# sholtodouglas/RoboticsPlayroomPybullet

Measured on AMD Instinct MI355X. Metric: env-steps/sec at N=4096 parallel UR5PlayAbsRPY1Obj-v0 envs per MI355X, higher is better.
Workload: dtype f32

## Files before the change

### roboticsplayroompybullet_amd/csrc/rp_kernels.cuh

```cuda
#pragma once
#include <hip/hip_runtime.h>
#include <stdint.h>

#include "rp_device_model.h"
#include "rp_math.cuh"

#define NB_MAX (1 + RP_MAX_ARM + RP_MAX_FREE + RP_MAX_J1)
#define NVP 28
#define MAXC 21
#define MAXACT 64
#define MAXT 4
#define MAXROWC (3 * MAXC + MAXT)
static_assert(MAXACT <= 64 && NB_MAX <= 32, "a candidate record packs its pair index in 6 bits and its bodies in 5 bits each");
#define PM_MAX 11
#define PMC_HDR 4
#define PMC_PT 11
#define PMC_MAN (8 + 4 * PMC_PT)
#define PMC_MANIFOLDS (PMC_HDR + PM_MAX * PMC_MAN)
#define PMC_AX PMC_MANIFOLDS
#define PMC_AXN 16
#define PMC_FLOATS (PMC_MANIFOLDS + 8 * PMC_AXN)
#define RP_MAX_GROUPS 16
#define SORT_KEYS 64
#define SORT_REPS 8
#define SORT_BINS (SORT_KEYS * SORT_REPS)
#define SORT_RANK_BITS 22
#define SORT_RANK_MASK ((1 << SORT_RANK_BITS) - 1)
#define RP_MAX_ENVS (1 << SORT_RANK_BITS)
#define MAXSMALL 44

#ifndef RP_PREP_WAVES
#define RP_PREP_WAVES 4
#endif
// ... 116 lines not shown
  };
  HULL_POOL_FIELDS
#ifdef RP_LDS_PAD
  float pad[RP_LDS_PAD];
#endif
};
static_assert(offsetof(EnvLds, aabb) % 16 == 0 && offsetof(PrepLds, aabb) % 16 == 0 && offsetof(EnvLds, cand) % 16 == 0 && offsetof(EnvLds, man) % 16 == 0 && offsetof(EnvLds, srow) % 16 == 0 && offsetof(EnvLds, rowS) % 16 == 0 &&
              offsetof(EnvLds, rowT) % 16 == 0 && offsetof(EnvLds, J) % 16 == 0 && offsetof(EnvLds, B) % 16 == 0, "16-byte LDS accesses");
static_assert(sizeof(PrepLds) <= 20480 - 512, "k_prep2: eight blocks (sixteen waves: what its 128 VGPRs allow) per CU");
static_assert(offsetof(PrepLds, roff) % 16 == 0 && offsetof(PrepLds, slot) % 16 == 0 && offsetof(PrepLds, Minv) % 16 == 0 && offsetof(PrepLds, aout) % 16 == 0 &&
              offsetof(PrepLds, Md) % 8 == 0 && offsetof(PrepLds, cand) % 16 == 0 && offsetof(PrepLds, man) % 16 == 0, "16-byte copies out of LDS");
static_assert(offsetof(PrepLds, rowS) % 16 == 0 && offsetof(PrepLds, rowT) % 16 == 0 && offsetof(PrepLds, J) % 8 == 0 && offsetof(PrepLds, B) % 8 == 0 && ROWW % 2 == 0,
              "prep2_core copies rowS / rowT a row (16 bytes) and J / B a pair (8 bytes) at a time");

struct __align__(16) ObsLds {
  float st[RP_REC_FLOATS];
  float xR[NB_MAX * 9], xp[NB_MAX * 3];
  float O[4];
  float S[RP_MAX_ARM * 6];
  alignas(16) float cand[2 * 12 * RP_MAX_ARM + 2 * RP_MAX_ARM + 4];
  alignas(16) float out[O_FLOATS];
};
#ifdef RP_CLOCKS
__device__ unsigned long long g_clk[32 * 4096];
#define CLK_MARK(i) if (lane == 0) { g_clk[8 * wb + (i)] = __builtin_readcyclecounter(); }
#if RP_CLOCKS == 2
#define PCLK(i) if (lane == 0) { g_clk[32 * (blockIdx.x & 4095) + (i)] = (i) >= 6 && (i) < 8 ? wall_clock64() : __builtin_readcyclecounter(); }
#define PCLK_ZERO(i) if (lane == 0) { g_clk[32 * (blockIdx.x & 4095) + (i)] = 0ull; }
#define PCLK_ADD(i, v) if (lane == 0) { g_clk[32 * (blockIdx.x & 4095) + (i)] += (unsigned long long)(v); }
#define HCLK_ADD(i, v) if (l16 == 0) { atomicAdd(&g_clk[32 * (blockIdx.x & 4095) + (i)], (unsigned long long)(v)); }
#ifdef RP_HPROF
#define PCLK_G(i, v)
#define PCLK_H(i, v) PCLK_ADD(i, v)
#else
#define PCLK_G(i, v) PCLK_ADD(i, v)
#define PCLK_H(i, v)
#endif
#define CLK_MARK2(i)
#else
#define PCLK(i)
#define PCLK_ZERO(i)
#define PCLK_ADD(i, v)
#define HCLK_ADD(i, v)
#define PCLK_G(i, v)
#define PCLK_H(i, v)
#define CLK_MARK2(i) CLK_MARK(i)
#endif
#else
#define CLK_MARK(i)
#define CLK_MARK2(i)
#define PCLK(i)
#define PCLK_ZERO(i)
#define PCLK_ADD(i, v)
#define HCLK_ADD(i, v)
#define PCLK_G(i, v)
#define PCLK_H(i, v)
#endif

#define WSYNC() do { __builtin_amdgcn_fence(__ATOMIC_RELEASE, "workgroup"); __builtin_amdgcn_wave_barrier(); __builtin_amdgcn_fence(__ATOMIC_ACQUIRE, "workgroup"); } while (0)

__device__ __forceinline__ int dof_free(const DevModel* m, int k) { return m->n_arm + 6 * k; }
__device__ __forceinline__ int dof_j1(const DevModel* m, int k) { return m->n_arm + 6 * m->n_free + k; }
#ifndef RP_WIDE
#define LANE_J1 16
#define LANE_FREE 19
__device__ __forceinline__ int lane_pos(const DevModel* m, int d) {
  if (d < m->n_arm) return d;
  const int e = d - m->n_arm, f6 = 6 * m->n_free;
  if (e >= f6) return LANE_J1 + (e - f6);
  const int f = e / 6, c = e - 6 * f;
  if ((m->free_row0 >> f) & 1) return c < 3 ? m->n_arm + c : -1;
  return LANE_FREE + e;
}
__device__ __forceinline__ int lane_dof(const DevModel* m, int l) {
  if (l < 16) {
    if (l < m->n_arm) return l;
// ... 70 lines not shown
  return x ^ (x >> 31);
}
__device__ __forceinline__ float rng_uniform(uint64_t seed, uint32_t env, uint32_t counter) {
  uint64_t h = splitmix64(seed ^ splitmix64(((uint64_t)env << 32) | counter));
  return (float)(h >> 40) * (1.0f / 16777216.0f);
}

struct Xf { M3 R; V3 p; };

__device__ __forceinline__ Xf joint_compose(const DevModel* m, const Xf& P, int j, float q) {
  Xf r;
  M3 Rj = mul(P.R, ldm3(m->arm_jrot[j]));
  r.p = P.p + mulv(P.R, ld3(m->arm_jpos[j]));
  V3 ax = ld3(m->arm_axis[j]);
  if (m->arm_jtype[j] == 0) {
    r.R = mul(Rj, axis_angle(ax, q));
  } else {
    r.R = Rj;
    r.p = r.p + mulv(Rj, ax) * q;
  }
  return r;
}

template <class LDS>
__device__ __forceinline__ void fk_bodies(const DevModel* m, LDS& L, int lane) {
  float* T = L.cand;
  static_assert(2 * 12 * RP_MAX_ARM + 2 * RP_MAX_ARM <= CANDMAX * 8 && 2 * 12 * RP_MAX_ARM + 2 * RP_MAX_ARM <= (int)(sizeof(L.cand) / sizeof(float)), "fk scratch fits the candidate list");
  int* P = (int*)(T + 2 * 12 * RP_MAX_ARM);
  const int n = m->n_arm;
  Xf x; x.R = ident3(); x.p = mk3(0, 0, 0);
  int par = -1;
  if (lane < n) {
    M3 R0 = ldm3(m->arm_jrot[lane]);
    V3 p0 = ld3(m->arm_jpos[lane]), ax = ld3(m->arm_axis[lane]);
    float q = L.st[ST_Q + lane];
    x.R = R0; x.p = p0;
    if (m->arm_jtype[lane] == 0) x.R = mul(R0, axis_angle(ax, q));
    else x.p = p0 + mulv(R0, ax) * q;
    par = m->arm_parent[lane];
    if (par < 0) { M3 Rb = ldm3(m->base_rot); V3 pb = ld3(m->base_pos); x.p = pb + mulv(Rb, x.p); x.R = mul(Rb, x.R); }
  }
  if (lane < m->nbody && !(lane >= 1 && lane <= n)) {
    int b = lane;
    Xf y; y.R = ident3(); y.p = mk3(0, 0, 0);
    if (b > n && b <= n + m->n_free) {
      int k = b - 1 - n;
      const float* f = &L.st[ST_FREE + 13 * k];
      Q4 q = {f[3], f[4], f[5], f[6]};
      y.R = quat_to_m3(q); y.p = ld3(f);
    } else if (b > n + m->n_free) {
      int k = b - 1 - n - m->n_free;
      M3 R0 = ldm3(m->j1_rot[k]);
      V3 ax = ld3(m->j1_axis[k]);
      y.p = ld3(m->j1_pos[k]);
      float q = L.st[ST_JQ + k];
      if (m->j1_type[k] == 0) y.R = mul(R0, axis_angle(ax, q));
      else { y.R = R0; y.p = y.p + mulv(R0, ax) * q; }
    }
    stm3(&L.xR[9 * b], y.R); st3(&L.xp[3 * b], y.p);
  }
  for (int it = 0; __ballot(par >= 0) != 0ull; it++) {
    float* Tb = T + (it & 1) * 12 * RP_MAX_ARM;
    int* Pb = P + (it & 1) * RP_MAX_ARM;
    if (lane < n) { stm3(&Tb[12 * lane], x.R); st3(&Tb[12 * lane + 9], x.p); Pb[lane] = par; }
    WSYNC();
    if (par >= 0) {
      M3 Ra = ldm3(&Tb[12 * par]); V3 pa = ld3(&Tb[12 * par + 9]);
      x.p = pa + mulv(Ra, x.p); x.R = mul(Ra, x.R);
      par = Pb[par];
    }
  }
  if (lane < n) { stm3(&L.xR[9 * (lane + 1)], x.R); st3(&L.xp[3 * (lane + 1)], x.p); }
}

template <class LDS>
__device__ __forceinline__ void joint_subspaces(const DevModel* m, LDS& L, int lane) {
  if (lane == 0) st3(L.O, ld3(&L.xp[3 * m->site_body[RP_SITE_EE]]));
  WSYNC();
  if (lane < m->n_arm) {
    V3 O = ld3(L.O);
    M3 R = ldm3(&L.xR[9 * (1 + lane)]);
    V3 a = mulv(R, ld3(m->arm_axis[lane]));
    V6 S;
    if (m->arm_jtype[lane] == 0) { S.a = a; S.l = cross(ld3(&L.xp[3 * (1 + lane)]) - O, a); }
    else { S.a = mk3(0, 0, 0); S.l = a; }
    st6(&L.S[6 * lane], S);
  }
}

template <class LDS>
__device__ __forceinline__ void stage_dynamics(const DevModel* m, LDS& L, int t, int env) {
  const int no = m->n_obj, nd = no + m->n_free;
  if (t < nd) {
    const float v = m->dyn[(size_t)env * nd + t];
    if (t < no) L.dmu[t] = v; else L.dmass[t - no] = v;
  }
}
template <class LDS>
__device__ __forceinline__ float pair_friction(const DevModel* m, const LDS& L, int a, int b) {
  return fminf(L.dmu[m->col_obj[a]] * L.dmu[m->col_obj[b]], 10.f);
}
__device__ __forceinline__ V3 ld_wrench(const DevModel* m, int env, int body, int half) {
  return ld3(m->wrench + ((size_t)env * (m->nbody - 1) + body) * 6 + 3 * half);
}
__device__ __forceinline__ bool wrench_on(V3 w) { return w.x != 0.f || w.y != 0.f || w.z != 0.f; }
__device__ __forceinline__ V3 ld_gravity(const DevModel* m, int env) { return ld3(m->act + (size_t)env * (3 + 2 * m->n_arm)); }
__device__ __forceinline__ float ld_motor_gain(const DevModel* m, int env, int dof) { return m->act[(size_t)env * (3 + 2 * m->n_arm) + 3 + dof]; }
__device__ __forceinline__ float ld_motor_strength(const DevModel* m, int env, int dof) { return m->act[(size_t)env * (3 + 2 * m->n_arm) + 3 + m->n_arm + dof]; }
template <class LDS>
__device__ __forceinline__ Xf collider_xf(const DevModel* m, const LDS& L, int c) {
  int b = m->col_body[c];
  M3 Rb = ldm3(&L.xR[9 * b]);
  Xf x;
  x.R = mul(Rb, ldm3(m->col_rot[c]));
  x.p = ld3(&L.xp[3 * b]) + mulv(Rb, ld3(m->col_pos[c]));
  return x;
}

template <class LDS>
__device__ __forceinline__ void collider_aabbs(const DevModel* m, LDS& L, int lane) {
  if (lane < m->n_col) {
    Xf x = collider_xf(m, L, lane);
    V3 he = ld3(m->col_he[lane]);
    float e[3];
    for (int i = 0; i < 3; i++)
      e[i] = m->col_type[lane] == 0 ? fabsf(x.R.m[3 * i]) * he.x + fabsf(x.R.m[3 * i + 1]) * he.y + fabsf(x.R.m[3 * i + 2]) * he.z : he.x;
    *(float4*)&L.aabb[8 * lane] = make_float4(x.p.x - e[0], x.p.y - e[1], x.p.z - e[2], m->col_margin[lane]);
    *(float4*)&L.aabb[8 * lane + 4] = make_float4(x.p.x + e[0], x.p.y + e[1], x.p.z + e[2], 0.f);
  }
}

struct CPt { V3 p, n; float dist; };

__device__ __forceinline__ int sphere_box(V3 cs, float r, V3 cb, const M3& Rb, V3 hb, float margin, int sphere_is_b, CPt* out) {
  const V3 l = tmulv(Rb, cs - cb);
  V3 cl = l;
  bool inside = true;
  if (cl.x > hb.x) { cl.x = hb.x; inside = false; }
  if (cl.x < -hb.x) { cl.x = -hb.x; inside = false; }
  if (cl.y > hb.y) { cl.y = hb.y; inside = false; }
  if (cl.y < -hb.y) { cl.y = -hb.y; inside = false; }
  if (cl.z > hb.z) { cl.z = hb.z; inside = false; }
  if (cl.z < -hb.z) { cl.z = -hb.z; inside = false; }
  V3 nl; float dist;
  if (!inside) {
    const V3 df = cl - l;
    const float len = norm(df);
    dist = len - r;
    if (dist > margin) return 0;
    nl = df * (1.f / len);
  } else {
    const float px = hb.x - fabsf(l.x), py = hb.y - fabsf(l.y), pz = hb.z - fabsf(l.z);
// ... 616 lines not shown
          pt.p = pB + nrm * (0.5f * dcon); pt.n = flip ? -nrm : nrm; pt.dist = dcon;
        }
        if (l16 == 0) {
          L.hout[gi] = out;
          if (out == 1) {
            float* q = &L.hpt[gi][0];
            st3(q, pt.p); st3(q + 3, pt.n); q[6] = pt.dist;
          }
        }
  }
}

template <class LDS>
__device__ __forceinline__ int narrowphase_coop(const DevModel* m, LDS& L, int lane, int nact, float* __restrict__ gax) {
  const int g = lane >> 3, s = lane & 7;
  float* scr = &L.npscr[NPG_SCRATCH * g];
  float* sv = scr;
  float (*poly)[8][3] = (float (*)[8][3])(scr + 16);
  float (*kept)[4] = (float (*)[4])(scr + 64);
  const unsigned below = (1u << s) - 1u;
  {
    const int ai = lane;
    const bool act = ai < nact;
    const int pi = act ? L.act[ai] : 0;
    const int a = m->pair[pi][0], b = m->pair[pi][1];
    const int ta = m->col_type[a], tb = m->col_type[b];
    const float margin0 = fminf(m->col_margin[a], m->col_margin[b]);
    int hf = -1;
      const int body_b0 = m->col_body[b], body_a0 = m->col_body[a];
      const bool hswap = act && m->hull_cnt[b] > 0 && ta == 0 && tb == 0 && body_a0 > m->n_arm;
      const int hc = hswap ? b : a, bc = hswap ? a : b;
      const int hn = act ? m->hull_cnt[hc] : 0;
      bool hq = hn > 0 && (hswap || (tb == 0 && body_b0 == 0));
      if (hq) {
        const Xf xa = collider_xf(m, L, hc), xb = collider_xf(m, L, bc);
        const V3 ha = ld3(m->col_he[hc]), hb0 = ld3(m->col_he[bc]);
        const V3 hb = mk3(fmaxf(hb0.x, RP_HULL_MARGIN), fmaxf(hb0.y, RP_HULL_MARGIN), fmaxf(hb0.z, RP_HULL_MARGIN));
        const V3 tt = xa.p - xb.p;
        const V3 A0 = col(xa.R, 0), A1 = col(xa.R, 1), A2 = col(xa.R, 2), B0 = col(xb.R, 0), B1 = col(xb.R, 1), B2 = col(xb.R, 2);
        const float r0 = ha.x * fabsf(dot(B0, A0)) + ha.y * fabsf(dot(B0, A1)) + ha.z * fabsf(dot(B0, A2));
        const float r1 = ha.x * fabsf(dot(B1, A0)) + ha.y * fabsf(dot(B1, A1)) + ha.z * fabsf(dot(B1, A2));
        const float r2 = ha.x * fabsf(dot(B2, A0)) + ha.y * fabsf(dot(B2, A1)) + ha.z * fabsf(dot(B2, A2));
        const float og = fmaxf(fmaxf(fabsf(dot(B0, tt)) - r0 - hb.x, fabsf(dot(B1, tt)) - r1 - hb.y), fabsf(dot(B2, tt)) - r2 - hb.z);
        const float q0 = hb.x * fabsf(dot(A0, B0)) + hb.y * fabsf(dot(A0, B1)) + hb.z * fabsf(dot(A0, B2));
        const float q1 = hb.x * fabsf(dot(A1, B0)) + hb.y * fabsf(dot(A1, B1)) + hb.z * fabsf(dot(A1, B2));
        const float q2 = hb.x * fabsf(dot(A2, B0)) + hb.y * fabsf(dot(A2, B1)) + hb.z * fabsf(dot(A2, B2));
        const float og2 = fmaxf(fmaxf(fabsf(dot(A0, tt)) - q0 - ha.x, fabsf(dot(A1, tt)) - q1 - ha.y), fabsf(dot(A2, tt)) - q2 - ha.z);
        if (fmaxf(og, og2) > margin0 + RP_HULL_MARGIN + 1e-5f) { hq = false; hf = 0; }
      }
      if (act) L.hout[ai] = hf;
      if (hq) { L.hinfo[ai][0] = hc | (bc << 8) | (hswap ? 65536 : 0); L.hinfo[ai][1] = __float_as_int(margin0); L.hinfo[ai][2] = pi; }
      const unsigned long long any = __ballot(hq);
      if (any != 0ull) {
        PCLK_H(30, -(long long)__builtin_readcyclecounter())
        const int slot = (gax && m->gjk) ? (pi & (PMC_AXN - 1)) : (ai & (PMC_AXN - 1));
        unsigned leaders = 0u;
        unsigned long long mycls = 0ull;
#pragma unroll 1
        for (int c = 0; c < PMC_AXN; c++) {
          const unsigned long long mk = __ballot(hq && slot == c);
          if (mk != 0ull) leaders |= 1u << c;
          if (lane == c) mycls = mk;
        }
        if (lane < PMC_AXN) L.hcls[lane] = mycls;
        WSYNC();
        {
          const int row = lane >> 4;
#pragma unroll 1
          for (unsigned rest = leaders; rest != 0u;) {
            unsigned t = rest;
            if (row >= 1) t &= t - 1u;
            if (row >= 2) t &= t - 1u;
            if (row >= 3) t &= t - 1u;
            unsigned long long cm = t != 0u ? L.hcls[__ffs(t) - 1] : 0ull;
            rest &= rest - 1u; rest &= rest - 1u; rest &= rest - 1u; rest &= rest - 1u;
#pragma unroll 1
            while (__any(cm != 0ull)) {
              const int gi = cm != 0ull ? __ffsll((long long)cm) - 1 : -1;
              cm &= cm - 1ull;
              hull_item16(m, L, lane, gi, gax);
            }
          }
        }
        PCLK_H(30, __builtin_readcyclecounter())
      }
    WSYNC();
    PCLK(19)
  }
  int cbase = 0;
  for (int base = 0; base < nact; base += 64 / NPG) {
    const int ai = base + g;
    const bool act = ai < nact;
    const int pi = act ? L.act[ai] : 0;
    const int a = m->pair[pi][0], b = m->pair[pi][1];
    const int ta = m->col_type[a], tb = m->col_type[b];
    const float margin0 = fminf(m->col_margin[a], m->col_margin[b]);
    const bool bbox = act && ta == 0 && tb == 0;
    if (act && s == 0) {
      const int n = m->n_arm, ba = m->col_body[a], bdy = m->col_body[b];
      const int kf = ba - 1 - n;
      const bool single = kf >= 0 && kf < m->n_free && m->free_rot_locked[kf] && bdy == 0;
      auto half0 = [&](int q) { int f = q - 1 - n; return q >= 1 && (q <= n || (f < m->n_free && ((m->free_row0 >> f) & 1))); };
      const bool r0 = half0(ba) || half0(bdy), r1 = (ba >= 1 && !half0(ba)) || (bdy >= 1 && !half0(bdy));
      const bool arm = (ba >= 1 && ba <= n) || (bdy >= 1 && bdy <= n), movable = ba > n || bdy > n;
      L.key[ai] = m->col_obj[a] * 256 + m->col_obj[b] + (single ? 65536 : 0) + ((r0 ? (r1 ? 2 : 1) : 0) << 20) + ((arm && movable) ? (1 << 22) : 0);
      L.pmu[ai] = pair_friction(m, L, a, b);
    }
    const int hf = act ? L.hout[ai] : -1;
    int np = 0;
    CPt mine; mine.p = mk3(0, 0, 0); mine.n = mk3(0, 0, 0); mine.dist = 0.f;
    if (hf == 1 && s == 0) { const float* hp = &L.hpt[ai][0]; mine.p = ld3(hp); mine.n = ld3(hp + 3); mine.dist = hp[6]; np = 1; }
    asm volatile("" ::: "memory");
    const Xf xa = collider_xf(m, L, a), xb = collider_xf(m, L, b);
    const V3 ha = ld3(m->col_he[a]), hb = ld3(m->col_he[b]);
    const bool bb = bbox && hf < 0;
    const int body_a = m->col_body[a], body_b = m->col_body[b];
    const bool arm_pair = (body_a >= 1 && body_a <= m->n_arm) || (body_b >= 1 && body_b <= m->n_arm);
    const float margin = (bb && (arm_pair || m->persist) && m->boxbox_margin >= 0.f) ? m->boxbox_margin : margin0;
    if (act && !bb && s == 0) {
      if (ta == 0 && tb == 1) np = sphere_box(xb.p, hb.x, xa.p, xa.R, ha, margin, 1, &mine);
      else if (ta == 1 && tb == 0) np = sphere_box(xa.p, ha.x, xb.p, xb.R, hb, margin, 0, &mine);
    }
    const V3 ca = xa.p, cb = xb.p;
    const V3 A0 = col(xa.R, 0), A1 = col(xa.R, 1), A2 = col(xa.R, 2), B0 = col(xb.R, 0), B1 = col(xb.R, 1), B2 = col(xb.R, 2);
    const V3 t = ca - cb;
    auto axis = [&](int ax, bool& valid) {
      valid = true;
      if (ax < 3) return pick3(ax, A0, A1, A2);
      if (ax < 6) return pick3(ax - 3, B0, B1, B2);
      int e = ax - 6, i = e / 3, j = e - 3 * i;
      V3 c = cross(pick3(i, A0, A1, A2), pick3(j, B0, B1, B2));
      float l = norm(c);
      valid = !(l < 1e-6f);
      return c * (1.f / l);
    };
#pragma unroll
    for (int round = 0; round < 2; round++) {
      int ax = 8 * round + s;
      if (bb && ax < 15) {
        bool valid;
        V3 Lx = axis(ax, valid);
        float ra = 0.f, rb = 0.f;
        ra += ha.x * fabsf(dot(Lx, A0)); rb += hb.x * fabsf(dot(Lx, B0));
        ra += ha.y * fabsf(dot(Lx, A1)); rb += hb.y * fabsf(dot(Lx, B1));
        ra += ha.z * fabsf(dot(Lx, A2)); rb += hb.z * fabsf(dot(Lx, B2));
        float sval = fabsf(dot(t, Lx)) - ra - rb;
        sv[ax] = valid ? sval : -1e30f;
      }
    }
    WSYNC();
    bool reject = !bb;
    float best_s = -1e30f, edge_s = -1e30f; int best_f = 0, ee = 0;
    if (bb) {
#pragma unroll
      for (int f = 0; f < 6; f++) {
        float sf = sv[f];
        reject |= sf > margin;
        if (sf > best_s + (f == 0 ? 0.f : K_TIE_EPS)) { best_s = sf; best_f = f; }
      }
#pragma unroll
      for (int e = 0; e < 9; e++) {
        float se = sv[6 + e];
        reject |= se > margin;
        if (se > edge_s + K_TIE_EPS) { edge_s = se; ee = e; }
      }
    }
    const bool live = bb && !reject;
    const bool edge_case = live && edge_s > best_s + 0.05f * fabsf(best_s) + 1e-6f;
    const bool face_case = live && !edge_case;
    const int best_kind = best_f < 3 ? 0 : 1, best_i = best_f < 3 ? best_f : best_f - 3;
    if (edge_case && s == 0) {
// ... 161 lines not shown
  return best;
}

__device__ __forceinline__ int solver_place(const int kept, const int pk, const unsigned long long lower, int& cls, int& before) {
  int key = 0, total = 0;
  cls = 0; before = 0;
  if (kept > 0) { cls = (pk >> 20) & 3; key = 2 * (cls == 2 ? 1 : 0) + ((pk >> 22) & 1); }
  unsigned long long mk[4];
#pragma unroll
  for (int k = 0; k < 4; k++) mk[k] = __ballot(kept > 0 && key == k);
#pragma unroll
  for (int bit = 0; bit < 3; bit++) {
    const unsigned long long mb = __ballot((kept >> bit) & 1);
    total += __popcll(mb) << bit;
#pragma unroll
    for (int k = 0; k < 4; k++) {
      const int all = __popcll(mb & mk[k]) << bit, low = __popcll(mb & mk[k] & lower) << bit;
      before += k < key ? all : (k == key ? low : 0);
    }
  }
  return total;
}

template <class LDS>
__device__ __forceinline__ int collide(const DevModel* m, LDS& L, int lane, int env, const int* npm_early = nullptr) {
  int nact = 0;
  const int npair = m->n_pair;
  const unsigned short* pp = (const unsigned short*)m->pair;
  unsigned short pv[RP_MAX_PAIR / 64];
#pragma unroll
  for (int k = 0; k < RP_MAX_PAIR / 64; k++) { int pi = 64 * k + lane; pv[k] = pp[pi < npair ? pi : 0]; }
  unsigned ovbits = 0u;
#pragma unroll
  for (int k = 0; k < RP_MAX_PAIR / 64; k++) {
    int pi = 64 * k + lane;
    if (64 * k < npair && pi < npair) {
      int a = pv[k] & 255, b = pv[k] >> 8;
      const float4 alo = *(const float4*)&L.aabb[8 * a], ahi = *(const float4*)&L.aabb[8 * a + 4];
      const float4 blo = *(const float4*)&L.aabb[8 * b], bhi = *(const float4*)&L.aabb[8 * b + 4];
      const float margin = fminf(alo.w, blo.w);
      bool sep = (alo.x > bhi.x + margin) | (blo.x > ahi.x + margin) | (alo.y > bhi.y + margin) | (blo.y > ahi.y + margin) | (alo.z > bhi.z + margin) | (blo.z > ahi.z + margin);
      ovbits |= sep ? 0u : (1u << k);
    }
  }
#pragma unroll
  for (int k = 0; k < RP_MAX_PAIR / 64; k++) {
    if (64 * k >= npair) break;
    bool ov = (ovbits >> k) & 1u;
    unsigned long long mask = __ballot(ov);
    int before = __popcll(mask & ((1ull << lane) - 1ull));
    if (ov && nact + before < MAXACT) L.act[nact + before] = 64 * k + lane;
    nact += __popcll(mask);
    if (nact >= MAXACT) { nact = MAXACT; break; }
  }
  WSYNC();
  PCLK(8)
#if defined(RP_CLOCKS) && RP_CLOCKS == 2
  if (lane == 0) g_clk[32 * (blockIdx.x & 4095) + 12] = nact;
#endif
  const int ncand_all = uni(narrowphase_coop<LDS>(m, L, lane, nact, m->persist ? m->pmcache + (size_t)env * PMC_FLOATS + PMC_AX : nullptr));
  WSYNC();
  asm volatile("" : "+v"(lane));
  PCLK(9)
  const unsigned long long lower = (1ull << lane) - 1ull;
  int kept = 0, pk = 0, total = 0;
  float* man = L.man;
  if (m->persist) {
    float* C = L.npscr + 8 * MANPTS;
    static_assert(8 * MANPTS + PMC_MANIFOLDS <= NPSCR_FLOATS, "the staged contact cache lies behind L.man in the narrowphase scratch");
    float* g = m->pmcache + (size_t)env * PMC_FLOATS;
    const int npm_pre = min(max(uni(npm_early ? *npm_early : __float_as_int(g[0])), 0), PM_MAX);
    const int used_in = PMC_HDR + PMC_MAN * npm_pre;
    for (int i = lane * 4; i < used_in; i += 256) *(float4*)&C[i] = *(const float4*)&g[i];
    if (lane == 0) C[0] = __int_as_float(npm_pre);
    WSYNC();
    PCLK(21)
    int npm = uni(__float_as_int(C[0]));
    const int mykey = lane < npm ? __float_as_int(C[PMC_HDR + PMC_MAN * lane]) : -1;
    const int akey = L.key[lane < nact ? lane : 0];
    const int pkey = L.key[lane >= 1 && lane < nact ? lane - 1 : 0];
    bool steady;
// ... 14 lines not shown
    }
    if (!steady) {
      {
        WSYNC();
        int nk = 0;
        for (int j = 0; j < npm; j++)
          if ((keep >> j) & 1ull) {
            if (nk != j && lane < PMC_MAN) C[PMC_HDR + PMC_MAN * nk + lane] = C[PMC_HDR + PMC_MAN * j + lane];
            nk++;
          }
        npm = nk;
        WSYNC();
      }
      {
        const int objk = lane < nact ? (L.key[lane] & 0xFFFF) : -1;
        const bool first = lane < nact && (lane == 0 || (L.key[lane - 1] & 0xFFFF) != objk);
        const int mkey = __float_as_int(C[PMC_HDR + PMC_MAN * (lane < npm ? lane : 0)]);
        bool present = false;
        for (int j = 0; j < npm; j++) present |= __builtin_amdgcn_readlane(mkey, j) == objk;
        const bool isnew = first && !present;
        const unsigned long long mnew = __ballot(isnew);
        const int slot = npm + __popcll(mnew & lower);
        if (isnew && slot < PM_MAX) {
          const int pi = L.act[lane];
          float* M = &C[PMC_HDR + PMC_MAN * slot];
          M[0] = __int_as_float(objk); M[1] = __int_as_float(0);
          M[2] = fminf(m->col_margin[m->pair[pi][0]], m->col_margin[m->pair[pi][1]]);
          M[3] = __int_as_float(L.key[lane] >> 16);
          for (int t = 4; t < PMC_MAN; t++) M[t] = 0.f;
        }
        npm = min(PM_MAX, npm + (int)__popcll(mnew));
        WSYNC();
      }
    }
    PCLK(22)
    unsigned long long unmatched, mine = 0ull;
    {
      const int ncand = ncand_all;
      const bool isc = lane < ncand;
      const float* c = &L.cand[8 * (isc ? lane : 0)];
      const V3 p = ld3(c), nr = mk3(c[3], c[4], c[5]);
      const float dist = c[6];
      const int abw = __float_as_int(c[7]);
      const int objk = L.key[(abw >> 16) & 63] & 0xFFFF;
      const int ba = (abw >> 22) & 31, bb = (abw >> 27) & 31;
      const M3 RA = ldm3(&L.xR[9 * ba]), RB = ldm3(&L.xR[9 * bb]);
      const V3 xA = ld3(&L.xp[3 * ba]), xB = ld3(&L.xp[3 * bb]);
      const int mkey = steady ? mykey : __float_as_int(C[PMC_HDR + PMC_MAN * (lane < npm ? lane : 0)]);
      int mi = -1;
      for (int jm = 0; jm < npm; jm++) if (__builtin_amdgcn_readlane(mkey, jm) == objk) mi = jm;
// ... 178 lines not shown
        } else if (cnt < 4) dst = cnt++;
        else dst = manifold_replace_index(man, c);
        if (dst >= 0) { const float4 c0 = *(const float4*)c, c1 = *(const float4*)(c + 4); *(float4*)&man[8 * dst] = c0; *(float4*)&man[8 * dst + 4] = c1; }
      }
    }
  }
  WSYNC();
  int cls, before;
  total = solver_place(kept, pk, lower, cls, before);
  for (int i = 0; i < kept; i++) {
    const float4 c0 = *(const float4*)&man[8 * i], c1 = *(const float4*)&man[8 * i + 4];
    const int ab = __float_as_int(c1.w);
    const int o = before + i;
    L.conp[3 * o] = c0.x; L.conp[3 * o + 1] = c0.y; L.conp[3 * o + 2] = c0.z;
    L.conn[3 * o] = c0.w; L.conn[3 * o + 1] = c1.x; L.conn[3 * o + 2] = c1.y;
    L.cond[o] = c1.z;
    L.cona[o] = ab & 255; L.conb[o] = (ab >> 8) & 255; L.conk[o] = cls;
    L.conmu[o] = L.pmu[(ab >> 16) & 63];
  }
  }
  WSYNC();
  PCLK(10)
  return total;
}

template <class LDS>
__device__ __forceinline__ void arm_dynamics(const DevModel* m, LDS& L, int lane, int env) {
  int n = m->n_arm;
  V3 O = ld3(L.O);
  V3 wf = mk3(0, 0, 0), wt = mk3(0, 0, 0);
  if (lane < n) { wf = ld_wrench(m, env, lane, 0); wt = ld_wrench(m, env, lane, 1); }
  const V3 grav = ld_gravity(m, env);
  if (lane < n) {
    M3 R = ldm3(&L.xR[9 * (1 + lane)]);
    V3 c = ld3(&L.xp[3 * (1 + lane)]) + mulv(R, ld3(m->arm_com[lane])) - O;
    float mass = m->arm_mass[lane];
    M3 Ic = ldm3(m->arm_inertia[lane]);
    M3 Rt; for (int i = 0; i < 3; i++) for (int j = 0; j < 3; j++) Rt.m[3 * i + j] = R.m[3 * j + i];
    M3 Iw = mul(mul(R, Ic), Rt);
    float cc = dot(c, c);
    float* I = &L.inert[10 * lane];
    I[0] = mass; st3(I + 1, c * mass);
    I[4] = Iw.m[0] + mass * (cc - c.x * c.x); I[5] = Iw.m[4] + mass * (cc - c.y * c.y); I[6] = Iw.m[8] + mass * (cc - c.z * c.z);
    I[7] = Iw.m[1] - mass * c.x * c.y; I[8] = Iw.m[2] - mass * c.x * c.z; I[9] = Iw.m[5] - mass * c.y * c.z;
  }
  WSYNC();
// ... 1490 lines not shown
#define W3_B (W3_J + ROWREG)
#define W3_SROW (W3_B + ROWREG)
#define W3_FLOATS (W3_SROW + 4 + 8 * MAXSMALL)
#define STAGE_FLOATS (128 + 2 * ROWREG)
#define AOUT_FLOATS (160 + 8 + 20)
static_assert(W3_A % 4 == 0 && W3_ROWS % 4 == 0 && W3_ROWT % 4 == 0 && W3_ROFF % 4 == 0 && AOUT_FLOATS % 4 == 0 && W3_FLOATS % 4 == 0, "16-byte copies");
static_assert(W3_J % 2 == 0 && W3_B % 2 == 0, "8-byte copies of the compact rows");

#define HV_MAXC 14
#ifndef S4_SLOTS0
#define S4_SLOTS0 8
#endif
#ifndef S4_SLOTS1
#define S4_SLOTS1 8
#endif
__device__ __forceinline__ int hv_class(int nc, int nA, int nB, int nC) {
  const bool heavy = nC != 0 || nA > S4_SLOTS0 || nB > S4_SLOTS1;
  return !heavy ? 0 : (nc <= HV_MAXC ? 1 : 2);
}
#define PREP_THREADS 128
__device__ __forceinline__ void prep2_core(PrepLds& L, const DevModel* __restrict__ m, const float* __restrict__ state, float* __restrict__ ws, const int env, const int cenv,
                                           int* __restrict__ pair_tab, const int pair_idx, int* __restrict__ hv_cnt = nullptr, int* __restrict__ hv_list = nullptr, const int prep_flags = 0) {
  const int tid = threadIdx.x, wid = tid >> 6, lane = tid & 63;
  PCLK(6) PCLK(0) PCLK_ZERO(15) PCLK_ZERO(19) PCLK_ZERO(26) PCLK_ZERO(27) PCLK_ZERO(28) PCLK_ZERO(29) PCLK_ZERO(30) PCLK_ZERO(31)
  static_assert(RP_REC_FLOATS == PREP_THREADS, "one float of the record per thread");
  L.st[tid] = state[(size_t)env * RP_REC_FLOATS + tid];
  if (tid == 64) L.hdr[3] = pair_idx;
  if (tid == 64 && m->persist) L.hdr[2] = __float_as_int(m->pmcache[(size_t)cenv * PMC_FLOATS]);
  stage_dynamics(m, L, tid, cenv);
  __syncthreads();
  PCLK(16)
  if (wid == 0) fk_bodies(m, L, lane);
  __syncthreads();
  PCLK(17)
  float* w = ws + (size_t)env * W3_FLOATS;
  if (wid == 0) {
    collider_aabbs(m, L, lane);
    WSYNC();
    PCLK(1)
    int ncon = collide<PrepLds>(m, L, lane, cenv, &L.hdr[2]);
    ncon = uni(ncon);
#ifdef RP_ABL_MAXCON
    if (ncon > RP_ABL_MAXCON) ncon = RP_ABL_MAXCON;
#endif
    if (lane == 0) L.hdr[0] = ncon;
    PCLK(2)
  } else {
    joint_subspaces(m, L, lane);
    PCLK(18)
    arm_dynamics(m, L, lane, cenv);
    unconstrained_velocities(m, L, lane, cenv);
    PCLK(3)
    int nsmall = build_small_rows(m, L, lane, cenv, (prep_flags & 2) != 0);
    nsmall = uni(nsmall);
    for (int i = lane; i < AOUT_FLOATS; i += 64) L.aout[i] = 0.f;
    if (lane < 2) L.amask[lane] = 0u;
    if (lane == 2) L.amask[2] = (unsigned)nsmall;
    WSYNC();
    bool gear = false;
    if (lane < nsmall) {
      const float* s = &L.srow[8 * lane];
      int type = __float_as_int(s[0]), dA = __float_as_int(s[1]);
      float sg = s[2], rhs = s[3], dinv = s[4], lo = s[5], hi = s[6];
// ... 1653 lines not shown
```

### roboticsplayroompybullet_amd/csrc/rp_playroom.hip

```cpp
#include <hip/hip_runtime.h>
#include <stdio.h>
#include <stdlib.h>
#include <string.h>

#include <vector>

#include "../../include/rp_playroom.h"
#include "../../include/rp_playroom_debug.h"
#include "generated/rp_models_gen.h"
#include "generated/rp_hullverts_gen.h"
#include "generated/rp_hullcells_gen.h"
#include "generated/rp_hullplanes_gen.h"
#include "rp_device_model.h"
#include "rp_kernels.cuh"
#include "rp_render.cuh"
#include "rp_closest.cuh"


static_assert(sizeof(RpViewEntry) == 128, "RpViewEntry is a by-value kernel argument: its layout must not move");

struct RpImageConfig {
  int n, n_fin, tiles, ftiles;
  RpViewTable obs, fin;
  int fmap[RC_MAX_VIEWS];
// ... 1440 lines not shown
    host_buf[2 * e + 1] = hdr[3] + 1000 * ((hdr[4] + hdr[7]) > 0) + 100000 * hdr[7];
  }
  return RP_OK;
}

#ifdef RP_PROLOGUE_CLOCKS
int rp_debug_prologue_clocks(rp_handle h, uint64_t* host_buf, int32_t nwaves) {
  if (!h || !host_buf || nwaves > 4096) return RP_ERR_ARG;
  HIPCHK(h, hipDeviceSynchronize());
  HIPCHK(h, hipMemcpyFromSymbol(host_buf, HIP_SYMBOL(g_pclk), (size_t)nwaves * 8 * sizeof(uint64_t)));
  return RP_OK;
}
#endif
#ifdef RP_CHAIN_CLOCKS
int rp_debug_chain_clocks(rp_handle h, int64_t* host_buf, int32_t nblocks) {
  if (!h || !host_buf || nblocks > 4096) return RP_ERR_ARG;
  HIPCHK(h, hipDeviceSynchronize());
  HIPCHK(h, hipMemcpyFromSymbol(host_buf, HIP_SYMBOL(g_chain_clk), (size_t)nblocks * 4 * sizeof(int64_t)));
  return RP_OK;
}
#endif
#ifdef RP_CLOCKS
#if RP_CLOCKS == 2
#define RP_CLK_STRIDE 32
#else
#define RP_CLK_STRIDE 8
#endif
int rp_debug_clocks(rp_handle h, uint64_t* host_buf, int32_t nblocks) {
  if (!h || !host_buf || nblocks > 4096) return RP_ERR_ARG;
  HIPCHK(h, hipDeviceSynchronize());
  HIPCHK(h, hipMemcpyFromSymbol(host_buf, HIP_SYMBOL(g_clk), (size_t)nblocks * RP_CLK_STRIDE * sizeof(uint64_t)));
  return RP_OK;
}
#endif

}
```

Baseline: 2.146 million.

## Prefetch model tables into registers at prep start and pack collider ids into active-pair entries

Wave 0 of prep2 now loads the pair list, its collider row and its FK joint row from the device model at kernel entry, alongside the state-record load, so these global-memory latencies overlap the dynamics stage instead of stalling fk, aabb and collide later. Active-pair entries now pack both collider indices next to the pair index, which removes the dependent m->pair lookup in the narrowphase. Each narrowphase group loads a full collider row once, and the pair-key and friction computation moves after the SAT work. Pair friction is computed inline from L.dmu. Holding the prefetched rows raises VGPR pressure in wave 0, and more profiling clock slots are added.

```diff
diff --git a/roboticsplayroompybullet_amd/csrc/rp_kernels.cuh b/roboticsplayroompybullet_amd/csrc/rp_kernels.cuh
--- a/roboticsplayroompybullet_amd/csrc/rp_kernels.cuh
+++ b/roboticsplayroompybullet_amd/csrc/rp_kernels.cuh
@@ -9,6 +9,11 @@
 #define NVP 28
 #define MAXC 21
 #define MAXACT 64
+#define ACT_AB 10
+#define ACT_PAIR(e) ((e) & ((1 << ACT_AB) - 1))
+#define ACT_A(e) (((e) >> ACT_AB) & 255)
+#define ACT_B(e) (((e) >> (ACT_AB + 8)) & 255)
+static_assert(RP_MAX_PAIR <= (1 << ACT_AB) && RP_MAX_COL <= 256, "an active-pair entry: 10 bits of pair index, 8 bits per collider");
 #define MAXT 4
 #define MAXROWC (3 * MAXC + MAXT)
 static_assert(MAXACT <= 64 && NB_MAX <= 32, "a candidate record packs its pair index in 6 bits and its bodies in 5 bits each");
@@ -171,13 +176,15 @@
   alignas(16) float out[O_FLOATS];
 };
 #ifdef RP_CLOCKS
-__device__ unsigned long long g_clk[32 * 4096];
+#define PCLK_STRIDE 40
+__device__ unsigned long long g_clk[PCLK_STRIDE * 4096];
 #define CLK_MARK(i) if (lane == 0) { g_clk[8 * wb + (i)] = __builtin_readcyclecounter(); }
 #if RP_CLOCKS == 2
-#define PCLK(i) if (lane == 0) { g_clk[32 * (blockIdx.x & 4095) + (i)] = (i) >= 6 && (i) < 8 ? wall_clock64() : __builtin_readcyclecounter(); }
-#define PCLK_ZERO(i) if (lane == 0) { g_clk[32 * (blockIdx.x & 4095) + (i)] = 0ull; }
-#define PCLK_ADD(i, v) if (lane == 0) { g_clk[32 * (blockIdx.x & 4095) + (i)] += (unsigned long long)(v); }
-#define HCLK_ADD(i, v) if (l16 == 0) { atomicAdd(&g_clk[32 * (blockIdx.x & 4095) + (i)], (unsigned long long)(v)); }
+#define PCLK(i) if (lane == 0) { g_clk[PCLK_STRIDE * (blockIdx.x & 4095) + (i)] = (i) >= 6 && (i) < 8 ? wall_clock64() : __builtin_readcyclecounter(); }
+#define PCLK_ZERO(i) if (lane == 0) { g_clk[PCLK_STRIDE * (blockIdx.x & 4095) + (i)] = 0ull; }
+#define PCLK_ADD(i, v) if (lane == 0) { g_clk[PCLK_STRIDE * (blockIdx.x & 4095) + (i)] += (unsigned long long)(v); }
+#define HCLK_ADD(i, v) if (l16 == 0) { atomicAdd(&g_clk[PCLK_STRIDE * (blockIdx.x & 4095) + (i)], (unsigned long long)(v)); }
+#define PCLK_HERE(x) asm volatile("" :: "v"(x));
 #ifdef RP_HPROF
 #define PCLK_G(i, v)
 #define PCLK_H(i, v) PCLK_ADD(i, v)
@@ -190,6 +197,7 @@
 #define PCLK(i)
 #define PCLK_ZERO(i)
 #define PCLK_ADD(i, v)
+#define PCLK_HERE(x)
 #define HCLK_ADD(i, v)
 #define PCLK_G(i, v)
 #define PCLK_H(i, v)
@@ -201,6 +209,7 @@
 #define PCLK(i)
 #define PCLK_ZERO(i)
 #define PCLK_ADD(i, v)
+#define PCLK_HERE(x)
 #define HCLK_ADD(i, v)
 #define PCLK_G(i, v)
 #define PCLK_H(i, v)
@@ -317,8 +326,20 @@
   return r;
 }
 
+struct FkRow { M3 rot; V3 pos, axis; int type, parent; };
+__device__ __forceinline__ FkRow ld_fk_row(const DevModel* m, int lane) {
+  const int n = m->n_arm, k = lane - 1 - n - m->n_free;
+  const bool arm = lane < n, j1 = !arm && k >= 0 && lane < m->nbody;
+  const int i = arm ? lane : (j1 ? k : 0);
+  FkRow r;
+  r.rot = ldm3(arm ? m->arm_jrot[i] : m->j1_rot[i]); r.pos = ld3(arm ? m->arm_jpos[i] : m->j1_pos[i]); r.axis = ld3(arm ? m->arm_axis[i] : m->j1_axis[i]);
+  r.type = *(arm ? &m->arm_jtype[i] : &m->j1_type[i]);
+  const int par = m->arm_parent[arm ? i : 0];
+  r.parent = arm ? par : -1;
+  return r;
+}
 template <class LDS>
-__device__ __forceinline__ void fk_bodies(const DevModel* m, LDS& L, int lane) {
+__device__ __forceinline__ void fk_bodies(const DevModel* m, LDS& L, int lane, const FkRow& row) {
   float* T = L.cand;
   static_assert(2 * 12 * RP_MAX_ARM + 2 * RP_MAX_ARM <= CANDMAX * 8 && 2 * 12 * RP_MAX_ARM + 2 * RP_MAX_ARM <= (int)(sizeof(L.cand) / sizeof(float)), "fk scratch fits the candidate list");
   int* P = (int*)(T + 2 * 12 * RP_MAX_ARM);
@@ -326,13 +347,13 @@
   Xf x; x.R = ident3(); x.p = mk3(0, 0, 0);
   int par = -1;
   if (lane < n) {
-    M3 R0 = ldm3(m->arm_jrot[lane]);
-    V3 p0 = ld3(m->arm_jpos[lane]), ax = ld3(m->arm_axis[lane]);
+    M3 R0 = row.rot;
+    V3 p0 = row.pos, ax = row.axis;
     float q = L.st[ST_Q + lane];
     x.R = R0; x.p = p0;
-    if (m->arm_jtype[lane] == 0) x.R = mul(R0, axis_angle(ax, q));
+    if (row.type == 0) x.R = mul(R0, axis_angle(ax, q));
     else x.p = p0 + mulv(R0, ax) * q;
-    par = m->arm_parent[lane];
+    par = row.parent;
     if (par < 0) { M3 Rb = ldm3(m->base_rot); V3 pb = ld3(m->base_pos); x.p = pb + mulv(Rb, x.p); x.R = mul(Rb, x.R); }
   }
   if (lane < m->nbody && !(lane >= 1 && lane <= n)) {
@@ -345,11 +366,11 @@
       y.R = quat_to_m3(q); y.p = ld3(f);
     } else if (b > n + m->n_free) {
       int k = b - 1 - n - m->n_free;
-      M3 R0 = ldm3(m->j1_rot[k]);
-      V3 ax = ld3(m->j1_axis[k]);
-      y.p = ld3(m->j1_pos[k]);
+      M3 R0 = row.rot;
+      V3 ax = row.axis;
+      y.p = row.pos;
       float q = L.st[ST_JQ + k];
-      if (m->j1_type[k] == 0) y.R = mul(R0, axis_angle(ax, q));
+      if (row.type == 0) y.R = mul(R0, axis_angle(ax, q));
       else { y.R = R0; y.p = y.p + mulv(R0, ax) * q; }
     }
     stm3(&L.xR[9 * b], y.R); st3(&L.xp[3 * b], y.p);
@@ -367,6 +388,8 @@
   }
   if (lane < n) { stm3(&L.xR[9 * (lane + 1)], x.R); st3(&L.xp[3 * (lane + 1)], x.p); }
 }
+template <class LDS>
+__device__ __forceinline__ void fk_bodies(const DevModel* m, LDS& L, int lane) { fk_bodies(m, L, lane, ld_fk_row(m, lane)); }
 
 template <class LDS>
 __device__ __forceinline__ void joint_subspaces(const DevModel* m, LDS& L, int lane) {
@@ -412,17 +435,37 @@
   return x;
 }
 
+struct ColRow { int body, type, obj; float margin; M3 rot; V3 pos, he; };
+__device__ __forceinline__ ColRow ld_collider(const DevModel* m, int c) {
+  ColRow r;
+  r.body = m->col_body[c]; r.type = m->col_type[c]; r.obj = m->col_obj[c]; r.margin = m->col_margin[c];
+  r.rot = ldm3(m->col_rot[c]); r.pos = ld3(m->col_pos[c]); r.he = ld3(m->col_he[c]);
+  return r;
+}
+template <class LDS>
+__device__ __forceinline__ Xf collider_xf(const LDS& L, const ColRow& c) {
+  M3 Rb = ldm3(&L.xR[9 * c.body]);
+  Xf x;
+  x.R = mul(Rb, c.rot);
+  x.p = ld3(&L.xp[3 * c.body]) + mulv(Rb, c.pos);
+  return x;
+}
+
+template <class LDS>
+__device__ __forceinline__ void collider_aabbs(const DevModel* m, LDS& L, int lane, const ColRow& c) {
+  if (lane < m->n_col) {
+    Xf x = collider_xf(L, c);
+    V3 he = c.he;
+    float e[3];
+    for (int i = 0; i < 3; i++)
+      e[i] = c.type == 0 ? fabsf(x.R.m[3 * i]) * he.x + fabsf(x.R.m[3 * i + 1]) * he.y + fabsf(x.R.m[3 * i + 2]) * he.z : he.x;
+    *(float4*)&L.aabb[8 * lane] = make_float4(x.p.x - e[0], x.p.y - e[1], x.p.z - e[2], c.margin);
+    *(float4*)&L.aabb[8 * lane + 4] = make_float4(x.p.x + e[0], x.p.y + e[1], x.p.z + e[2], 0.f);
+  }
+}
 template <class LDS>
 __device__ __forceinline__ void collider_aabbs(const DevModel* m, LDS& L, int lane) {
-  if (lane < m->n_col) {
-    Xf x = collider_xf(m, L, lane);
-    V3 he = ld3(m->col_he[lane]);
-    float e[3];
-    for (int i = 0; i < 3; i++)
-      e[i] = m->col_type[lane] == 0 ? fabsf(x.R.m[3 * i]) * he.x + fabsf(x.R.m[3 * i + 1]) * he.y + fabsf(x.R.m[3 * i + 2]) * he.z : he.x;
-    *(float4*)&L.aabb[8 * lane] = make_float4(x.p.x - e[0], x.p.y - e[1], x.p.z - e[2], m->col_margin[lane]);
-    *(float4*)&L.aabb[8 * lane + 4] = make_float4(x.p.x + e[0], x.p.y + e[1], x.p.z + e[2], 0.f);
-  }
+  collider_aabbs(m, L, lane, ld_collider(m, lane < m->n_col ? lane : 0));
 }
 
 struct CPt { V3 p, n; float dist; };
@@ -1085,16 +1128,17 @@
   {
     const int ai = lane;
     const bool act = ai < nact;
-    const int pi = act ? L.act[ai] : 0;
-    const int a = m->pair[pi][0], b = m->pair[pi][1];
+    const int ae = act ? L.act[ai] : 0;
+    const int pi = ACT_PAIR(ae), a = ACT_A(ae), b = ACT_B(ae);
     const int ta = m->col_type[a], tb = m->col_type[b];
     const float margin0 = fminf(m->col_margin[a], m->col_margin[b]);
     int hf = -1;
       const int body_b0 = m->col_body[b], body_a0 = m->col_body[a];
-      const bool hswap = act && m->hull_cnt[b] > 0 && ta == 0 && tb == 0 && body_a0 > m->n_arm;
+      const int hna = m->hull_cnt[a], hnb = m->hull_cnt[b];
+      const bool hswap = act & (hnb > 0) & (ta == 0) & (tb == 0) & (body_a0 > m->n_arm);
       const int hc = hswap ? b : a, bc = hswap ? a : b;
-      const int hn = act ? m->hull_cnt[hc] : 0;
-      bool hq = hn > 0 && (hswap || (tb == 0 && body_b0 == 0));
+      const int hn = act ? (hswap ? hnb : hna) : 0;
+      bool hq = (hn > 0) & (hswap | ((tb == 0) & (body_b0 == 0)));
       if (hq) {
         const Xf xa = collider_xf(m, L, hc), xb = collider_xf(m, L, bc);
         const V3 ha = ld3(m->col_he[hc]), hb0 = ld3(m->col_he[bc]);
@@ -1112,6 +1156,7 @@
         if (fmaxf(og, og2) > margin0 + RP_HULL_MARGIN + 1e-5f) { hq = false; hf = 0; }
       }
       if (act) L.hout[ai] = hf;
+      PCLK(33)
       if (hq) { L.hinfo[ai][0] = hc | (bc << 8) | (hswap ? 65536 : 0); L.hinfo[ai][1] = __float_as_int(margin0); L.hinfo[ai][2] = pi; }
       const unsigned long long any = __ballot(hq);
       if (any != 0ull) {
@@ -1152,32 +1197,28 @@
   }
   int cbase = 0;
   for (int base = 0; base < nact; base += 64 / NPG) {
+    PCLK_ADD(34, -(long long)__builtin_readcyclecounter()) PCLK_ADD(36, -(long long)__builtin_readcyclecounter()) PCLK_ADD(35, 1)
     const int ai = base + g;
     const bool act = ai < nact;
-    const int pi = act ? L.act[ai] : 0;
-    const int a = m->pair[pi][0], b = m->pair[pi][1];
-    const int ta = m->col_type[a], tb = m->col_type[b];
-    const float margin0 = fminf(m->col_margin[a], m->col_margin[b]);
+    const int ae = act ? L.act[ai] : 0;
+    const int a = ACT_A(ae), b = ACT_B(ae);
+    PCLK_HERE(a) PCLK_HERE(b) PCLK_ADD(36, __builtin_readcyclecounter())
+    const ColRow rowa = ld_collider(m, a), rowb = ld_collider(m, b);
+    const int ta = rowa.type, tb = rowb.type;
+    const float margin0 = fminf(rowa.margin, rowb.margin);
     const bool bbox = act && ta == 0 && tb == 0;
-    if (act && s == 0) {
-      const int n = m->n_arm, ba = m->col_body[a], bdy = m->col_body[b];
-      const int kf = ba - 1 - n;
-      const bool single = kf >= 0 && kf < m->n_free && m->free_rot_locked[kf] && bdy == 0;
-      auto half0 = [&](int q) { int f = q - 1 - n; return q >= 1 && (q <= n || (f < m->n_free && ((m->free_row0 >> f) & 1))); };
-      const bool r0 = half0(ba) || half0(bdy), r1 = (ba >= 1 && !half0(ba)) || (bdy >= 1 && !half0(bdy));
-      const bool arm = (ba >= 1 && ba <= n) || (bdy >= 1 && bdy <= n), movable = ba > n || bdy > n;
-      L.key[ai] = m->col_obj[a] * 256 + m->col_obj[b] + (single ? 65536 : 0) + ((r0 ? (r1 ? 2 : 1) : 0) << 20) + ((arm && movable) ? (1 << 22) : 0);
-      L.pmu[ai] = pair_friction(m, L, a, b);
-    }
+    const int kfree = rowa.body - 1 - m->n_arm;
+    const int rot_locked = m->free_rot_locked[(kfree >= 0 && kfree < m->n_free) ? kfree : 0];
     const int hf = act ? L.hout[ai] : -1;
     int np = 0;
     CPt mine; mine.p = mk3(0, 0, 0); mine.n = mk3(0, 0, 0); mine.dist = 0.f;
     if (hf == 1 && s == 0) { const float* hp = &L.hpt[ai][0]; mine.p = ld3(hp); mine.n = ld3(hp + 3); mine.dist = hp[6]; np = 1; }
     asm volatile("" ::: "memory");
-    const Xf xa = collider_xf(m, L, a), xb = collider_xf(m, L, b);
-    const V3 ha = ld3(m->col_he[a]), hb = ld3(m->col_he[b]);
+    const Xf xa = collider_xf(L, rowa), xb = collider_xf(L, rowb);
+    const V3 ha = rowa.he, hb = rowb.he;
+    PCLK_HERE(xa.R.m[8]) PCLK_HERE(xa.p.z) PCLK_HERE(xb.R.m[8]) PCLK_HERE(xb.p.z) PCLK_ADD(34, __builtin_readcyclecounter())
     const bool bb = bbox && hf < 0;
-    const int body_a = m->col_body[a], body_b = m->col_body[b];
+    const int body_a = rowa.body, body_b = rowb.body;
     const bool arm_pair = (body_a >= 1 && body_a <= m->n_arm) || (body_b >= 1 && body_b <= m->n_arm);
     const float margin = (bb && (arm_pair || m->persist) && m->boxbox_margin >= 0.f) ? m->boxbox_margin : margin0;
     if (act && !bb && s == 0) {
@@ -1210,6 +1251,15 @@
         float sval = fabsf(dot(t, Lx)) - ra - rb;
         sv[ax] = valid ? sval : -1e30f;
       }
+    }
+    if (act && s == 0) {
+      const int n = m->n_arm, ba = body_a, bdy = body_b;
+      const bool single = kfree >= 0 && kfree < m->n_free && rot_locked && bdy == 0;
+      auto half0 = [&](int q) { int f = q - 1 - n; return q >= 1 && (q <= n || (f < m->n_free && ((m->free_row0 >> f) & 1))); };
+      const bool r0 = half0(ba) || half0(bdy), r1 = (ba >= 1 && !half0(ba)) || (bdy >= 1 && !half0(bdy));
+      const bool arm = (ba >= 1 && ba <= n) || (bdy >= 1 && bdy <= n), movable = ba > n || bdy > n;
+      L.key[ai] = rowa.obj * 256 + rowb.obj + (single ? 65536 : 0) + ((r0 ? (r1 ? 2 : 1) : 0) << 20) + ((arm && movable) ? (1 << 22) : 0);
+      L.pmu[ai] = fminf(L.dmu[rowa.obj] * L.dmu[rowb.obj], 10.f);
     }
     WSYNC();
     bool reject = !bb;
@@ -1417,14 +1467,21 @@
   return total;
 }
 
+struct PairList { unsigned short pv[RP_MAX_PAIR / 64]; };
+__device__ __forceinline__ PairList ld_pair_list(const DevModel* m, int lane) {
+  const int npair = m->n_pair;
+  const unsigned short* pp = (const unsigned short*)m->pair;
+  PairList r;
+#pragma unroll
+  for (int k = 0; k < RP_MAX_PAIR / 64; k++) { int pi = 64 * k + lane; r.pv[k] = pp[pi < npair ? pi : 0]; }
+  return r;
+}
 template <class LDS>
-__device__ __forceinline__ int collide(const DevModel* m, LDS& L, int lane, int env, const int* npm_early = nullptr) {
+__device__ __forceinline__ int collide(const DevModel* m, LDS& L, int lane, int env, const int* npm_early, const PairList& plist) {
   int nact = 0;
   const int npair = m->n_pair;
-  const unsigned short* pp = (const unsigned short*)m->pair;
-  unsigned short pv[RP_MAX_PAIR / 64];
-#pragma unroll
-  for (int k = 0; k < RP_MAX_PAIR / 64; k++) { int pi = 64 * k + lane; pv[k] = pp[pi < npair ? pi : 0]; }
+  const unsigned short (&pv)[RP_MAX_PAIR / 64] = plist.pv;
+  PCLK_HERE(pv[RP_MAX_PAIR / 64 - 1]) PCLK(32)
   unsigned ovbits = 0u;
 #pragma unroll
   for (int k = 0; k < RP_MAX_PAIR / 64; k++) {
@@ -1444,14 +1501,14 @@
     bool ov = (ovbits >> k) & 1u;
     unsigned long long mask = __ballot(ov);
     int before = __popcll(mask & ((1ull << lane) - 1ull));
-    if (ov && nact + before < MAXACT) L.act[nact + before] = 64 * k + lane;
+    if (ov && nact + before < MAXACT) L.act[nact + before] = (64 * k + lane) | ((int)pv[k] << ACT_AB);
     nact += __popcll(mask);
     if (nact >= MAXACT) { nact = MAXACT; break; }
   }
   WSYNC();
   PCLK(8)
 #if defined(RP_CLOCKS) && RP_CLOCKS == 2
-  if (lane == 0) g_clk[32 * (blockIdx.x & 4095) + 12] = nact;
+  if (lane == 0) g_clk[PCLK_STRIDE * (blockIdx.x & 4095) + 12] = nact;
 #endif
   const int ncand_all = uni(narrowphase_coop<LDS>(m, L, lane, nact, m->persist ? m->pmcache + (size_t)env * PMC_FLOATS + PMC_AX : nullptr));
   WSYNC();
@@ -1512,10 +1569,10 @@
         const unsigned long long mnew = __ballot(isnew);
         const int slot = npm + __popcll(mnew & lower);
         if (isnew && slot < PM_MAX) {
-          const int pi = L.act[lane];
+          const int ae = L.act[lane];
           float* M = &C[PMC_HDR + PMC_MAN * slot];
           M[0] = __int_as_float(objk); M[1] = __int_as_float(0);
-          M[2] = fminf(m->col_margin[m->pair[pi][0]], m->col_margin[m->pair[pi][1]]);
+          M[2] = fminf(m->col_margin[ACT_A(ae)], m->col_margin[ACT_B(ae)]);
           M[3] = __int_as_float(L.key[lane] >> 16);
           for (int t = 4; t < PMC_MAN; t++) M[t] = 0.f;
         }
@@ -1740,6 +1797,10 @@
   WSYNC();
   PCLK(10)
   return total;
+}
+template <class LDS>
+__device__ __forceinline__ int collide(const DevModel* m, LDS& L, int lane, int env, const int* npm_early = nullptr) {
+  return collide<LDS>(m, L, lane, env, npm_early, ld_pair_list(m, lane));
 }
 
 template <class LDS>
@@ -3276,23 +3337,26 @@
 __device__ __forceinline__ void prep2_core(PrepLds& L, const DevModel* __restrict__ m, const float* __restrict__ state, float* __restrict__ ws, const int env, const int cenv,
                                            int* __restrict__ pair_tab, const int pair_idx, int* __restrict__ hv_cnt = nullptr, int* __restrict__ hv_list = nullptr, const int prep_flags = 0) {
   const int tid = threadIdx.x, wid = tid >> 6, lane = tid & 63;
-  PCLK(6) PCLK(0) PCLK_ZERO(15) PCLK_ZERO(19) PCLK_ZERO(26) PCLK_ZERO(27) PCLK_ZERO(28) PCLK_ZERO(29) PCLK_ZERO(30) PCLK_ZERO(31)
+  PCLK(6) PCLK(0) PCLK_ZERO(15) PCLK_ZERO(19) PCLK_ZERO(26) PCLK_ZERO(27) PCLK_ZERO(28) PCLK_ZERO(29) PCLK_ZERO(30) PCLK_ZERO(31) PCLK_ZERO(34) PCLK_ZERO(35) PCLK_ZERO(36)
   static_assert(RP_REC_FLOATS == PREP_THREADS, "one float of the record per thread");
-  L.st[tid] = state[(size_t)env * RP_REC_FLOATS + tid];
+  const float st_t = state[(size_t)env * RP_REC_FLOATS + tid];
+  FkRow fkrow = {}; ColRow crow = {}; PairList plist = {};
+  if (wid == 0) { plist = ld_pair_list(m, lane); crow = ld_collider(m, lane < m->n_col ? lane : 0); fkrow = ld_fk_row(m, lane); }
+  L.st[tid] = st_t;
   if (tid == 64) L.hdr[3] = pair_idx;
   if (tid == 64 && m->persist) L.hdr[2] = __float_as_int(m->pmcache[(size_t)cenv * PMC_FLOATS]);
   stage_dynamics(m, L, tid, cenv);
   __syncthreads();
   PCLK(16)
-  if (wid == 0) fk_bodies(m, L, lane);
+  if (wid == 0) { PCLK_HERE(fkrow.rot.m[8]) PCLK_HERE(fkrow.pos.z) PCLK_HERE(fkrow.axis.z) PCLK_HERE(fkrow.parent) PCLK(20) fk_bodies(m, L, lane, fkrow); }
   __syncthreads();
   PCLK(17)
   float* w = ws + (size_t)env * W3_FLOATS;
   if (wid == 0) {
-    collider_aabbs(m, L, lane);
+    collider_aabbs(m, L, lane, crow);
     WSYNC();
     PCLK(1)
-    int ncon = collide<PrepLds>(m, L, lane, cenv, &L.hdr[2]);
+    int ncon = collide<PrepLds>(m, L, lane, cenv, &L.hdr[2], plist);
     ncon = uni(ncon);
 #ifdef RP_ABL_MAXCON
     if (ncon > RP_ABL_MAXCON) ncon = RP_ABL_MAXCON;
diff --git a/roboticsplayroompybullet_amd/csrc/rp_playroom.hip b/roboticsplayroompybullet_amd/csrc/rp_playroom.hip
--- a/roboticsplayroompybullet_amd/csrc/rp_playroom.hip
+++ b/roboticsplayroompybullet_amd/csrc/rp_playroom.hip
@@ -1486,7 +1486,7 @@
 #endif
 #ifdef RP_CLOCKS
 #if RP_CLOCKS == 2
-#define RP_CLK_STRIDE 32
+#define RP_CLK_STRIDE PCLK_STRIDE
 #else
 #define RP_CLK_STRIDE 8
 #endif
```

New measurement: 2.162 million (median of 6 runs). About the same (+0.7%).
